# secondmind-labs/markovflow

Hardware: AMD Instinct MI355X
Metric: Kalman log-lik steps/sec (BxT) at d=6 (higher is better)
Workload: dtype f64; 1 GPU; KalmanFilter.log_likelihood B=1024/GPU T=10000 d=6 m=1 f64 (sum of two Matern-5/2, north-star target config); series_per_gpu=1024, state_dim=6, output_dim=1, parallelism=batch-sharded x1, one scalar RCCL all-reduce

## Files before the change

### markovflow_amd/csrc/mf_head_carry.hpp

```cpp
#pragma once

namespace mf {

template <int ROWB, int UNIT, typename Keep> struct HeadCarry {
    static constexpr int LINE = 128;
    static constexpr int MAXT = 2;
    static constexpr int UG = (ROWB + UNIT - 1) / UNIT;
    static constexpr int STEP = ROWB % LINE;
    static constexpr int cand(int t) {
        int n = 0;
        for (int u = 0; u < UG; ++u)
            if (Keep::keep(u, UNIT) && (u + 1) * UNIT <= LINE - 4) { if (n == t) return u; ++n; }
        return -1;
    }
    static constexpr int count_cand() { int n = 0; while (n < MAXT && cand(n) >= 0) ++n; return n; }
    static constexpr int tail_index(int u) { for (int t = 0; t < count_cand(); ++t) if (cand(t) == u) return t; return -1; }
    static constexpr unsigned carried_units(int r) {
        r &= LINE - 1;
        if (r == 0) return 0u;
        const int room = LINE - r;
        unsigned m = 0u;
        for (int u = 0; u < UG; ++u) {
            if (!Keep::keep(u, UNIT) || u * UNIT >= room) continue;
            const int t = tail_index(u);
            if (t < 0 || (u + 1) * UNIT > room) return 0u;
            m |= 1u << t;
        }
        return m;
    }
    static constexpr unsigned table(int t) {
        unsigned m = 0u;
        for (int g = 0; g < 32; ++g) if ((carried_units(4 * g) >> t) & 1u) m |= 1u << g;
        return m;
    }
    static constexpr unsigned TAB0 = table(0), TAB1 = table(1);
    static constexpr int period() { int p = 1, r = STEP; while (r % LINE) { r += STEP; ++p; } return p; }
    static constexpr int PERIOD = (ROWB % 4 == 0) ? period() : 0;
    static constexpr bool USABLE = ROWB % 4 == 0 && ROWB >= LINE && STEP != 0 && Keep::keep(UG - 1, UNIT) && (TAB0 | TAB1) != 0u;
    static constexpr int NT = USABLE ? count_cand() : 0;
    static constexpr int tail_unit(int t) { return cand(t); }

    static constexpr bool carried(unsigned addr, int t) { return (((t == 0 ? TAB0 : TAB1) >> ((addr & (LINE - 1)) >> 2)) & 1u) != 0u; }

    static constexpr unsigned consumer_bits(unsigned addr0) {
        unsigned m = 0u;
        for (int t = 0; t < NT; ++t)
            for (int p = 0; p < PERIOD; ++p) if (carried(addr0 + (unsigned)(p * STEP), t)) m |= 1u << (t * PERIOD + p);
        return m;
    }
    static constexpr unsigned producer_bits(unsigned addr0, int kind) {
        unsigned m = 0u;
        for (int p = 0; p < PERIOD; ++p) {
            bool f = true;
            if (kind >= 1 + MAXT) f = carried(addr0 + (unsigned)((p + 1) * STEP), kind - 1 - MAXT);
            else if (kind >= 1) f = !carried(addr0 + (unsigned)(p * STEP), kind - 1);
            if (f) m |= 1u << p;
        }
        return m;
    }
};

template <int ROWB, typename Keep, bool TAIL = false> struct Stream {
    static constexpr int UNIT = (ROWB >= 16) ? 16 : 4;
    static constexpr int UG = (ROWB + UNIT - 1) / UNIT;
    static constexpr int count_kept() { int n = 0; for (int u = 0; u < UG; ++u) n += Keep::keep(u, UNIT) ? 1 : 0; return n; }
    using HC = HeadCarry<ROWB, UNIT, Keep>;
    static constexpr int UB = count_kept();
    static constexpr int NT = TAIL ? HC::NT : 0;
    static constexpr int U = UB + NT;
    static constexpr int NI = U;
    static constexpr int LDS_BYTES = 64 * U * UNIT;
    static constexpr bool ALL = (UB == UG) && NT == 0;
    static constexpr int global_unit(int c) {
        int n = 0;
        for (int u = 0; u < UG; ++u) if (Keep::keep(u, UNIT)) { if (n == c) return u; ++n; }
        return -1;
    }
    static constexpr int global_offset(int c) { return c < UB ? global_unit(c) * UNIT : ROWB + HC::tail_unit(c - UB) * UNIT; }
    static constexpr int unit_kind(int c) {
        if (c >= UB) return 1 + HC::MAXT + (c - UB);
        for (int t = 0; t < NT; ++t) if (global_unit(c) == HC::tail_unit(t)) return 1 + t;
        return 0;
    }
    static constexpr int compact_unit(int gu) {
        int n = 0;
        for (int u = 0; u < gu; ++u) n += Keep::keep(u, UNIT) ? 1 : 0;
        return n;
    }
};

struct KeepAll { static constexpr bool keep(int, int) { return true; } };
template <int D, int S> struct KeepLower {
    static constexpr bool keep(int u, int unit) {
        const int lo = u * unit, hi = lo + unit;
        for (int i = 0; i < D; ++i) {
            const int a = (i * D) * S, b = (i * D + i + 1) * S;
            if (a < hi && lo < b) return true;
        }
        return false;
    }
};

}
```

### markovflow_amd/csrc/mf_kf_lds.hpp

```cpp
#pragma once
#include "mf_kernels.hpp"
#include "mf_head_carry.hpp"
#include <type_traits>
#ifndef MF_PUMPMASK
#define MF_PUMPMASK 63
#endif

namespace mf {

typedef int mf_v4i __attribute__((ext_vector_type(4)));

#define MF_POLICY_STR_0 ""
#define MF_POLICY_STR_1 " nt"
#define MF_POLICY_STR_2 " sc1"
#define MF_POLICY_STR_3 " sc0 sc1"
#define MF_POLICY_STR_4 " sc0"
#define MF_POLICY_CAT(n) MF_POLICY_STR_##n
#define MF_POLICY_OF(n) MF_POLICY_CAT(n)
#ifndef MF_POLW
#define MF_POLW 1
#endif
#ifndef MF_POLN
#define MF_POLN 0
#endif
#define MF_POLICY_WIDE MF_POLICY_OF(MF_POLW)
#define MF_POLICY_NARROW MF_POLICY_OF(MF_POLN)
#define MF_DMA_HEAD "s_nop 4\n\ts_mov_b32 %0, m0\n\ts_mov_b32 m0, %2\n\ts_nop 0\n\t"
#define MF_DMA_TAIL "s_mov_b32 m0, %0"
#define MF_DMA_X4(v, pol) "buffer_load_dwordx4 " v ", %1, 0 offen" pol " lds\n\t"
#define MF_DMA_X1(v, pol) "buffer_load_dword " v ", %1, 0 offen" pol " lds\n\t"
#define MF_DMA_STEP4 "s_add_u32 m0, m0, 0x400\n\ts_nop 0\n\t"
#define MF_DMA_STEP1 "s_add_u32 m0, m0, 0x100\n\ts_nop 0\n\t"
template <bool WIDE, int N> MF_DEV void dma_b128_group(mf_v4i srd, unsigned lds_addr, const unsigned* v) {
    unsigned keep;
    static_assert(N >= 1 && N <= 4, "group size");
#define MF_DMA_B128_BODY(POL)                                                                                                       \
    if constexpr (N == 1)                                                                                                           \
        asm volatile(MF_DMA_HEAD MF_DMA_X4("%3", POL) MF_DMA_TAIL : "=&s"(keep) : "s"(srd), "s"(lds_addr), "v"(v[0]) : "memory", "scc"); \
    else if constexpr (N == 2)                                                                                                      \
        asm volatile(MF_DMA_HEAD MF_DMA_X4("%3", POL) MF_DMA_STEP4 MF_DMA_X4("%4", POL) MF_DMA_TAIL                                 \
                     : "=&s"(keep) : "s"(srd), "s"(lds_addr), "v"(v[0]), "v"(v[1]) : "memory", "scc");                              \
    else if constexpr (N == 3)                                                                                                      \
        asm volatile(MF_DMA_HEAD MF_DMA_X4("%3", POL) MF_DMA_STEP4 MF_DMA_X4("%4", POL) MF_DMA_STEP4 MF_DMA_X4("%5", POL) MF_DMA_TAIL \
                     : "=&s"(keep) : "s"(srd), "s"(lds_addr), "v"(v[0]), "v"(v[1]), "v"(v[2]) : "memory", "scc");                   \
    else                                                                                                                            \
        asm volatile(MF_DMA_HEAD MF_DMA_X4("%3", POL) MF_DMA_STEP4 MF_DMA_X4("%4", POL) MF_DMA_STEP4 MF_DMA_X4("%5", POL)           \
                     MF_DMA_STEP4 MF_DMA_X4("%6", POL) MF_DMA_TAIL                                                                  \
                     : "=&s"(keep) : "s"(srd), "s"(lds_addr), "v"(v[0]), "v"(v[1]), "v"(v[2]), "v"(v[3]) : "memory", "scc");
    if (WIDE) { MF_DMA_B128_BODY(MF_POLICY_WIDE) } else { MF_DMA_B128_BODY(MF_POLICY_NARROW) }
#undef MF_DMA_B128_BODY
}
template <int N> MF_DEV void dma_b32_group(mf_v4i srd, unsigned lds_addr, const unsigned* v) {
    unsigned keep;
    static_assert(N >= 1 && N <= 4, "group size");
    if constexpr (N == 1)
        asm volatile(MF_DMA_HEAD MF_DMA_X1("%3", MF_POLICY_NARROW) MF_DMA_TAIL : "=&s"(keep) : "s"(srd), "s"(lds_addr), "v"(v[0]) : "memory", "scc");
    else if constexpr (N == 2)
        asm volatile(MF_DMA_HEAD MF_DMA_X1("%3", MF_POLICY_NARROW) MF_DMA_STEP1 MF_DMA_X1("%4", MF_POLICY_NARROW) MF_DMA_TAIL
                     : "=&s"(keep) : "s"(srd), "s"(lds_addr), "v"(v[0]), "v"(v[1]) : "memory", "scc");
    else if constexpr (N == 3)
        asm volatile(MF_DMA_HEAD MF_DMA_X1("%3", MF_POLICY_NARROW) MF_DMA_STEP1 MF_DMA_X1("%4", MF_POLICY_NARROW) MF_DMA_STEP1
                     MF_DMA_X1("%5", MF_POLICY_NARROW) MF_DMA_TAIL
                     : "=&s"(keep) : "s"(srd), "s"(lds_addr), "v"(v[0]), "v"(v[1]), "v"(v[2]) : "memory", "scc");
    else
        asm volatile(MF_DMA_HEAD MF_DMA_X1("%3", MF_POLICY_NARROW) MF_DMA_STEP1 MF_DMA_X1("%4", MF_POLICY_NARROW) MF_DMA_STEP1
                     MF_DMA_X1("%5", MF_POLICY_NARROW) MF_DMA_STEP1 MF_DMA_X1("%6", MF_POLICY_NARROW) MF_DMA_TAIL
                     : "=&s"(keep) : "s"(srd), "s"(lds_addr), "v"(v[0]), "v"(v[1]), "v"(v[2]), "v"(v[3]) : "memory", "scc");
}


constexpr unsigned MF_DMA_INVALID = 0xF0000000u;
constexpr unsigned long long MF_DMA_MAXREC = 0xE0000000ull;

template <typename St, typename = void> struct StreamTail { static constexpr int NT = 0, PERIOD = 1; };
template <typename St> struct StreamTail<St, std::enable_if_t<(St::NT > 0)>> { static constexpr int NT = St::NT, PERIOD = St::HC::PERIOD; };

template <typename St> struct DmaStream {
    using TL = StreamTail<St>;
    unsigned vo[St::NI];
    static constexpr int PB = TL::PERIOD;
    static constexpr int FW = TL::NT > 0 ? (St::NI * PB + 31) / 32 : 1;
    unsigned fm[FW];
    MF_DEV void init(const char* smem, int lane, int rel_tab, int gtab, unsigned base_lo = 0u) {
        const int q0 = lane / St::U, c0 = lane - q0 * St::U;
        if constexpr (TL::NT > 0) { MF_UNROLL for (int w = 0; w < FW; ++w) fm[w] = 0u; }
        MF_UNROLL for (int i = 0; i < St::NI; ++i) {
            const int a = (64 * i) / St::U, b = (64 * i) % St::U;
            int cu = c0 + b;
            const int carry = cu >= St::U ? 1 : 0;
            cu -= carry * St::U;
            const int row = q0 + a + carry;
            const unsigned rel = *reinterpret_cast<const unsigned*>(smem + rel_tab + row * 4);
            unsigned off;
            if (St::ALL) off = (unsigned)cu * St::UNIT;
            else off = *reinterpret_cast<const unsigned*>(smem + gtab + cu * 4);
            vo[i] = rel + off;
            if constexpr (TL::NT > 0) {
                static_assert(PB < 32 && 32 % PB == 0, "an instruction's schedule bits do not straddle two words");
                int kind = 0;
                MF_UNROLL for (int cc = 0; cc < St::U; ++cc) if (St::unit_kind(cc) != 0 && cu == cc) kind = St::unit_kind(cc);
                unsigned bits = (1u << PB) - 1u;
                MF_UNROLL for (int kk = 1; kk <= 2 * St::HC::MAXT; ++kk)
                    if (kind == kk) bits = St::HC::producer_bits(base_lo + rel, kk);
                fm[(i * PB) / 32] |= bits << ((i * PB) % 32);
            }
#ifdef MF_EXPERIMENT
            if (pack_base != 0xffffffffu && rel < MF_DMA_INVALID)
                vo[i] |= ((((pack_base + rel) >> 5) & 3u) << 29) | ((unsigned)(off / St::UNIT) << 24);
#endif
        }
    }
#ifdef MF_EXPERIMENT
    unsigned pack_base = 0xffffffffu;
    unsigned step_next = 0;
    bool skip_carried = false;
    MF_DEV unsigned exp_offset(unsigned v) const {
        if (pack_base == 0xffffffffu || v >= MF_DMA_INVALID) return v;
        const unsigned phase = ((v >> 29) + step_next) & 3u, gu = (v >> 24) & 31u, off = v & 0xffffffu;
        const bool carried = skip_carried && phase != 0u && gu < 8u - 2u * phase;
        return carried ? MF_DMA_INVALID : off;
    }
#endif
    template <int I0, int I1, bool SCHED = false> MF_DEV void issue(mf_v4i srd, unsigned lds_base, unsigned phase = 0u) const {
        constexpr int HI = I1 < St::NI ? I1 : St::NI;
        if constexpr (I0 < HI) {
            constexpr int N = (HI - I0) < 4 ? (HI - I0) : 4;
            unsigned voff[N];
            MF_UNROLL for (int k = 0; k < N; ++k) {
#ifdef MF_EXPERIMENT
                voff[k] = exp_offset(vo[I0 + k]);
#else
                voff[k] = vo[I0 + k];
#endif
                if constexpr (SCHED && TL::NT > 0)
                    voff[k] = ((fm[((I0 + k) * PB) / 32] >> (((I0 + k) * PB) % 32 + phase)) & 1u) ? voff[k] : MF_DMA_INVALID;
            }
            if (St::UNIT == 16) dma_b128_group<(St::UG >= 8), N>(srd, lds_base + I0 * 1024, voff);
            else dma_b32_group<N>(srd, lds_base + I0 * 256, voff);
            issue<I0 + N, I1, SCHED>(srd, lds_base, phase);
        }
    }
};

MF_DEV unsigned long long uniform64(unsigned long long x) {
    const unsigned lo = (unsigned)__builtin_amdgcn_readfirstlane((int)(unsigned)x);
    const unsigned hi = (unsigned)__builtin_amdgcn_readfirstlane((int)(unsigned)(x >> 32));
    return ((unsigned long long)hi << 32) | lo;
}

MF_DEV mf_v4i make_srd(unsigned long long base, unsigned long long end, int debug = 0) {
    unsigned long long rem = end > base ? end - base : 0ull;
    if (debug & 1) rem = 0;
    if (rem > MF_DMA_MAXREC) rem = MF_DMA_MAXREC;
    mf_v4i srd;
    srd.x = __builtin_amdgcn_readfirstlane((int)(unsigned)base);
    srd.y = __builtin_amdgcn_readfirstlane((int)((unsigned)(base >> 32) & 0xffffu));
    srd.z = __builtin_amdgcn_readfirstlane((int)(unsigned)rem);
    srd.w = 0x00020000;
    return srd;
}

template <typename T, typename St> struct RowReader {
    const char* row;
    MF_DEV RowReader(const char* smem, int lds_off, int lane) : row(smem + lds_off + lane * (St::U * St::UNIT)) {}
    MF_DEV T at(int e) const {
        const int byte = e * (int)sizeof(T);
        const int gu = byte / St::UNIT;
        const int off = St::compact_unit(gu) * St::UNIT + (byte - gu * St::UNIT);
        return *reinterpret_cast<const T*>(row + off);
    }
    MF_DEV T tail_at(int t, int k) const { return *reinterpret_cast<const T*>(row + (St::UB + t) * St::UNIT + k * (int)sizeof(T)); }
};

template <typename T, int D, int M, bool RSTEP = false, int BG = 1, bool CARRY = false> struct KfLdsCfg {
    static constexpr int S = sizeof(T);
    static constexpr int BGRP = BG;
    using StA = Stream<D * D * S, KeepAll>;
    using StC0 = Stream<D * D * S, KeepLower<D, S>>;
    using StCT = Stream<D * D * S, KeepLower<D, S>, true>;
    using Stb = Stream<BG * D * S, KeepAll>;
    using StH = Stream<BG * M * D * S, KeepAll>;
    static constexpr int YG = (M == 1) ? 4 : 1;
    using Sty = Stream<YG * M * S, KeepAll>;
    using StR = Stream<M * M * S, KeepAll>;
    static constexpr bool RS = RSTEP;
    static constexpr int QUARTER_CU = (160 * 1024) / 4;
    static constexpr int TABLE_BYTES = 5 * 256 + ((StCT::U * 4 + 15) / 16) * 16;
    static constexpr int IMAGE_T = StA::LDS_BYTES + StCT::LDS_BYTES + Stb::LDS_BYTES + StH::LDS_BYTES + ((Sty::LDS_BYTES + 15) / 16) * 16 +
                                   (RSTEP ? ((StR::LDS_BYTES + 15) / 16) * 16 : 0);
    static constexpr bool TAIL = CARRY && StCT::NT > 0 && !StC0::ALL && StCT::NI * StCT::HC::PERIOD <= 64 &&
                                 StCT::NT * StCT::HC::PERIOD <= 32 && IMAGE_T <= QUARTER_CU && TABLE_BYTES <= IMAGE_T &&
                                 (StA::NI + StCT::NI + Stb::NI + StH::NI + Sty::NI + (RSTEP ? StR::NI : 0)) < 64;
    using StC = Stream<D * D * S, KeepLower<D, S>, TAIL>;
    static constexpr int OFF_A = 0;
    static constexpr int OFF_C = OFF_A + StA::LDS_BYTES;
    static constexpr int OFF_b = OFF_C + StC::LDS_BYTES;
    static constexpr int OFF_H = OFF_b + Stb::LDS_BYTES;
    static constexpr int OFF_y = OFF_H + StH::LDS_BYTES;
    static constexpr int OFF_R = OFF_y + ((Sty::LDS_BYTES + 15) / 16) * 16;
    static constexpr int IMAGE_END = OFF_R + (RSTEP ? ((StR::LDS_BYTES + 15) / 16) * 16 : 0);
    static constexpr int OFF_relA = TAIL ? 0 : IMAGE_END;
    static constexpr int OFF_relb = OFF_relA + 256;
    static constexpr int OFF_relH = OFF_relb + 256;
    static constexpr int OFF_rely = OFF_relH + 256;
    static constexpr int OFF_relR = OFF_rely + 256;
    static constexpr int OFF_gtabC = OFF_relR + 256;
    static constexpr int LDS_TOTAL = TAIL ? IMAGE_END : OFF_gtabC + ((StC::U * 4 + 15) / 16) * 16;
    static constexpr bool SUPPORTED =
                                      (StA::NI + StC::NI + Stb::NI + StH::NI + Sty::NI + (RSTEP ? StR::NI : 0)) < 64 &&
                                      LDS_TOTAL <= 64 * 1024;
};

template <typename T, int D, int M, bool RSTEP = false> using KfChunkCfg = KfLdsCfg<T, D, M, RSTEP, 1, true>;
static_assert(KfChunkCfg<double, 6, 1>::TAIL && KfChunkCfg<double, 6, 1>::LDS_TOTAL <= 40960, "fp64 d = 6: four wavefronts per CU");

template <typename Cfg> struct KfPump {
    static constexpr int N_SMALL = Cfg::StC::NI + Cfg::Stb::NI + Cfg::StH::NI + Cfg::Sty::NI + (Cfg::RS ? Cfg::StR::NI : 0);
    static constexpr int N_BIG = Cfg::StA::NI;
    const DmaStream<typename Cfg::StA>& dA; const DmaStream<typename Cfg::StC>& dC;
    const DmaStream<typename Cfg::Stb>& db; const DmaStream<typename Cfg::StH>& dH;
    const DmaStream<typename Cfg::Sty>& dy; const DmaStream<typename Cfg::StR>& dR;
    mf_v4i sA, sC, sb, sH, sy, sR;
    unsigned lds0;
    bool more;
    bool yfetch = true;
    unsigned cphase = 0;
    template <int K> MF_DEV void small() const {
        if (!((MF_PUMPMASK >> K) & 1)) return;
        small_do<K>();
    }
    template <int K> MF_DEV void small_do() const {
        if (!more) return;
        constexpr int HC = (Cfg::StC::NI + 1) / 2;
        if (K == 0) dC.template issue<0, HC, true>(sC, lds0 + Cfg::OFF_C, cphase);
        else {
            dC.template issue<HC, 64, true>(sC, lds0 + Cfg::OFF_C, cphase);
            db.template issue<0, 64>(sb, lds0 + Cfg::OFF_b);
            dH.template issue<0, 64>(sH, lds0 + Cfg::OFF_H);
            if (yfetch) dy.template issue<0, 64>(sy, lds0 + Cfg::OFF_y);
            if (Cfg::RS) dR.template issue<0, 64>(sR, lds0 + Cfg::OFF_R);
        }
    }
    template <int K> MF_DEV void all() const {
        dC.template issue<0, 64>(sC, lds0 + Cfg::OFF_C);
        db.template issue<0, 64>(sb, lds0 + Cfg::OFF_b);
        dH.template issue<0, 64>(sH, lds0 + Cfg::OFF_H);
        dy.template issue<0, 64>(sy, lds0 + Cfg::OFF_y);
        if (Cfg::RS) dR.template issue<0, 64>(sR, lds0 + Cfg::OFF_R);
        dA.template issue<0, 64>(sA, lds0 + Cfg::OFF_A);
    }
    template <int K> MF_DEV void big() const {
        if (!((MF_PUMPMASK >> (K + 2)) & 1)) return;
        big_do<K>();
    }
    MF_DEV void unpumped() const {
        if (!((MF_PUMPMASK >> 0) & 1)) small_do<0>();
        if (!((MF_PUMPMASK >> 1) & 1)) small_do<1>();
        if (!((MF_PUMPMASK >> 2) & 1)) big_do<0>();
        if (!((MF_PUMPMASK >> 3) & 1)) big_do<1>();
        if (!((MF_PUMPMASK >> 4) & 1)) big_do<2>();
        if (!((MF_PUMPMASK >> 5) & 1)) big_do<3>();
    }
    template <int K> MF_DEV void big_do() const {
        if (!more) return;
        constexpr int Q = (Cfg::StA::NI + 3) / 4;
        dA.template issue<K * Q, (K + 1) * Q>(sA, lds0 + Cfg::OFF_A);
    }
};

template <typename T, int D, int M, bool SPIKE, bool FIRST, typename Pump>
MF_DEV void kf_lds_step(Elim<T, D, SPIKE>& E, LogAcc<T>& laC, T& acc_yry, T& acc_ww, const T (&C)[D][D],
                        const T (&mvec)[D], const T (&hk)[M * D], const T (&yk)[M], const T (&Rsh)[M * M],
                        T (&Bm)[D][D], const Pump& pump, bool active, bool sep_lane) {
    const bool sep = FIRST && sep_lane, ord = active && !sep;
    T Ci[D][D], w[D], btw[D];
    if (active) {
        tri_inv_lower<T, D>(C, Ci, laC, E.bad);
        laC.renorm();
    }
    pump.template small<0>();
    if (active) {
        trimul_lower_vec<T, D>(Ci, mvec, w);
        acc_ww += dot_self<T, D>(w);
    }
    pump.template small<1>();
    pump.template big<0>();
    if (active) {
        trimul_lower_inplace<T, D, D>(Ci, Bm);
        gemv_t<T, D, D>(Bm, w, btw);
    }
    pump.template big<1>();
    if (FIRST && active && sep) {
        syrk_tn_lower<T, D, D>(Bm, E.GU, T(1));
        MF_UNROLL for (int i = 0; i < D; ++i) E.gU[i] = -btw[i];
    }
    if (ord) {
        syrk_tn_lower<T, D, D>(Bm, E.Phi, T(1));
        MF_UNROLL for (int i = 0; i < D; ++i) E.t[i] -= btw[i];
    }
    pump.template big<2>();
    if (FIRST && active && sep) {
        neg_trimulT_lower_inplace<T, D, D>(Ci, Bm);
        MF_UNROLL for (int i = 0; i < D; ++i) MF_UNROLL for (int j = 0; j < D; ++j) E.X[i][j] = Bm[i][j];
    }
    if (ord) E.eliminate_main();
    pump.template big<3>();
    if (FIRST && active && sep) {
        trimulT_self_lower<T, D>(Ci, E.Phi);
        trimulT_lower_vec<T, D>(Ci, w, E.t);
        acc_yry += Obs<T, D, M>::apply(hk, yk, Rsh, M, E.Phi, E.t);
    }
    if (ord) {
        E.eliminate_spike();
        trsm_right_lower_t<T, D, D>(E.Phi, E.Li, Bm);
        neg_trimulT_lower_inplace<T, D, D>(Ci, Bm);
        T Dn[D][D], rn[D];
        trimulT_self_lower<T, D>(Ci, Dn);
        trimulT_lower_vec<T, D>(Ci, w, rn);
        acc_yry += Obs<T, D, M>::apply(hk, yk, Rsh, M, Dn, rn);
        E.advance(Bm, Dn, rn);
    }
}

template <typename T, int D, int M, bool SPIKE, bool RSTEP = false>
__global__ void __launch_bounds__(64) kf_chunk_lds_kernel(KfArgs<T> a, long L, RedSys<T> out) {
    using Cfg = KfChunkCfg<T, D, M, RSTEP>;
    extern __shared__ __attribute__((aligned(16))) char smem[];
    const int lane = threadIdx.x;
    const long total = a.B * a.P;
    const long id_raw = (long)blockIdx.x * 64 + lane;
    const bool valid = id_raw < total;
    const long id = valid ? id_raw : total - 1;
    const long s = id / a.P, c = id % a.P;
    const long nt = a.Tn - 1;
    const long tau0 = c * L;
    long len = nt - tau0;
    if (len > L) len = L;
    if (len < 0 || !valid) len = 0;
    constexpr int S = sizeof(T);

    const unsigned long long offA = (unsigned long long)(s * nt + tau0) * (D * D * S);
    const unsigned long long offb = (unsigned long long)(s * nt + tau0) * (D * S);
    const unsigned long long offH = (unsigned long long)(s * a.Tn + tau0 + 1) * (M * D * S);
    const unsigned long long offy = (unsigned long long)(s * a.Tn + tau0 + 1) * (M * S);
    const unsigned long long offR = (unsigned long long)(s * a.Tn + tau0 + 1) * (M * M * S);
    const unsigned long long offA0 = uniform64(offA), offb0 = uniform64(offb);
    const unsigned long long offH0 = uniform64(offH), offy0 = uniform64(offy), offR0 = uniform64(offR);
    const bool rowok = valid && len > 0;
    {
        unsigned* tab = reinterpret_cast<unsigned*>(smem);
        tab[Cfg::OFF_relA / 4 + lane] = rowok ? (unsigned)(offA - offA0) : MF_DMA_INVALID;
        tab[Cfg::OFF_relb / 4 + lane] = rowok ? (unsigned)(offb - offb0) : MF_DMA_INVALID;
        tab[Cfg::OFF_relH / 4 + lane] = rowok ? (unsigned)(offH - offH0) : MF_DMA_INVALID;
        tab[Cfg::OFF_rely / 4 + lane] = rowok ? (unsigned)(offy - offy0) : MF_DMA_INVALID;
        tab[Cfg::OFF_relR / 4 + lane] = rowok ? (unsigned)(offR - offR0) : MF_DMA_INVALID;
        if (lane < Cfg::StC::U) {
            unsigned g = 0;
            MF_UNROLL for (int cc = 0; cc < Cfg::StC::U; ++cc) if (lane == cc) g = (unsigned)Cfg::StC::global_offset(cc);
            tab[Cfg::OFF_gtabC / 4 + lane] = g;
        }
    }
    DmaStream<typename Cfg::StA> dA;
    DmaStream<typename Cfg::StC> dC;
    DmaStream<typename Cfg::Stb> db;
    DmaStream<typename Cfg::StH> dH;
    DmaStream<typename Cfg::Sty> dy;
    DmaStream<typename Cfg::StR> dR;
    unsigned long long pA = (unsigned long long)a.A + offA0, pC = (unsigned long long)a.cholQ + offA0;
    unsigned long long pb = (unsigned long long)a.b + offb0, pH = (unsigned long long)a.H + offH0;
    unsigned long long py = (unsigned long long)a.y + offy0;
    unsigned long long pR = (unsigned long long)a.Rinv + (RSTEP ? offR0 : 0ull);
    const unsigned long long eA = (unsigned long long)a.A + (unsigned long long)a.B * nt * (D * D * S);
    const unsigned long long eC = (unsigned long long)a.cholQ + (unsigned long long)a.B * nt * (D * D * S);
    const unsigned long long eb = (unsigned long long)a.b + (unsigned long long)a.B * nt * (D * S);
    const unsigned long long eH = (unsigned long long)a.H + (unsigned long long)a.B * a.Tn * (M * D * S);
    const unsigned long long ey = (unsigned long long)a.y + (unsigned long long)a.B * a.Tn * (M * S);
    const unsigned long long eR = (unsigned long long)a.Rinv + (RSTEP ? (unsigned long long)a.B * a.Tn * (M * M * S) : 0ull);
    const unsigned lds0 = (unsigned)(size_t)smem;

    Elim<T, D, SPIKE> E;
    E.init();
    LogAcc<T> laC;
    laC.init();
    T acc_yry = T(0), acc_ww = T(0);
    T Rsh[M * M];
    MF_UNROLL for (int i = 0; i < M * M; ++i) Rsh[i] = RSTEP ? (valid ? a.Rinv[(s * a.Tn) * M * M + i] : T(0)) : a.Rinv[i];
    if (valid && c == 0) {
        T C[D][D], Ci[D][D], mvec[D], w[D];
        load_lower<T, D>(a.cholP0 + s * D * D, C);
        load_vec<T, D>(a.mu0 + s * D, mvec);
        tri_inv_lower<T, D>(C, Ci, laC, E.bad);
        laC.renorm();
        trimul_lower_vec<T, D>(Ci, mvec, w);
        acc_ww += dot_self<T, D>(w);
        trimulT_self_lower<T, D>(Ci, E.Phi);
        trimulT_lower_vec<T, D>(Ci, w, E.t);
        acc_yry += Obs<T, D, M>::apply(a.H + (s * a.Tn) * M * D, a.y + (s * a.Tn) * M, Rsh, M, E.Phi, E.t);
    }

    long nsteps = len;
    MF_UNROLL for (int off = 32; off > 0; off >>= 1) {
        const long o = __shfl_xor((long long)nsteps, off);
        nsteps = o > nsteps ? o : nsteps;
    }
    nsteps = __builtin_amdgcn_readfirstlane((int)nsteps);
    asm volatile("s_waitcnt vmcnt(0) lgkmcnt(0)" ::: "memory");
#ifdef MF_EXPERIMENT
    if (a.debug & 8) {
        dA.pack_base = (unsigned)__builtin_amdgcn_readfirstlane((int)(unsigned)pA);
        dC.pack_base = (unsigned)__builtin_amdgcn_readfirstlane((int)(unsigned)pC);
    }
#endif
    dA.init(smem, lane, Cfg::OFF_relA, 0);
    dC.init(smem, lane, Cfg::OFF_relA, Cfg::OFF_gtabC, (unsigned)pC);
    db.init(smem, lane, Cfg::OFF_relb, 0);
    dH.init(smem, lane, Cfg::OFF_relH, 0);
    dy.init(smem, lane, Cfg::OFF_rely, 0);
    if (RSTEP) dR.init(smem, lane, Cfg::OFF_relR, 0);
    asm volatile("s_waitcnt lgkmcnt(0)" ::: "memory");
    using HC = typename Cfg::StC::HC;
    constexpr int NTAIL = Cfg::StC::NT, CPER = NTAIL > 0 ? HC::PERIOD : 1, UEL = Cfg::StC::UNIT / S;
    const unsigned cbits = NTAIL > 0 ? HC::consumer_bits((unsigned)((unsigned long long)a.cholQ + offA)) : 0u;
    T cv[NTAIL > 0 ? NTAIL : 1][UEL];
    MF_UNROLL for (int t = 0; t < (NTAIL > 0 ? NTAIL : 1); ++t) MF_UNROLL for (int k = 0; k < UEL; ++k) cv[t][k] = T(0);

    const RowReader<T, typename Cfg::StA> rA(smem, Cfg::OFF_A, lane);
    const RowReader<T, typename Cfg::StC> rC(smem, Cfg::OFF_C, lane);
    const RowReader<T, typename Cfg::Stb> rb(smem, Cfg::OFF_b, lane);
    const RowReader<T, typename Cfg::StH> rH(smem, Cfg::OFF_H, lane);
    const RowReader<T, typename Cfg::Sty> ry(smem, Cfg::OFF_y, lane);
    const RowReader<T, typename Cfg::StR> rR(smem, Cfg::OFF_R, lane);

    using Pump = KfPump<Cfg>;

    if (nsteps > 0) {
        Pump p0{dA, dC, db, dH, dy, dR, make_srd(pA, eA, a.debug), make_srd(pC, eC, a.debug | ((a.debug >> 2) & 1)),
                make_srd(pb, eb, a.debug | ((a.debug >> 1) & 1)), make_srd(pH, eH, a.debug | ((a.debug >> 1) & 1)),
                make_srd(py, ey, a.debug | ((a.debug >> 1) & 1)), make_srd(pR, eR, a.debug | ((a.debug >> 1) & 1)), lds0, true};
        p0.template all<0>();
    }

#ifdef MF_STAMP
#define MF_STAMP_AT(var) { unsigned long long t_; asm volatile("s_memtime %0\n\ts_waitcnt lgkmcnt(0)" : "=s"(t_) :: "memory"); var = t_; }
    unsigned long long st_wait = 0, st_io = 0, st_comp = 0, ts0 = 0, ts1 = 0, ts2 = 0, ts3 = 0;
#define MF_STAMP_ACC { asm volatile("" :: "v"(E.quad), "v"(E.Phi[0][0]) : "memory"); MF_STAMP_AT(ts3) st_wait += ts1 - ts0; st_io += ts2 - ts1; st_comp += ts3 - ts2; }
#else
#define MF_STAMP_AT(var)
#define MF_STAMP_ACC
#endif
#ifdef MF_CHECKSUM
    T cs_A = 0, cs_C = 0, cs_b = 0, cs_H = 0, cs_y = 0;
#define MF_CHECKSUM_ACC if (j < len) { MF_UNROLL for (int i = 0; i < D; ++i) { cs_b += mvec[i]; MF_UNROLL for (int jj = 0; jj < D; ++jj) { cs_A += Bm[i][jj] * T(1 + i * D + jj); if (jj <= i) cs_C += C[i][jj] * T(1 + i * D + jj); } } \
        MF_UNROLL for (int i = 0; i < M * D; ++i) cs_H += hk[i] * T(1 + i); MF_UNROLL for (int i = 0; i < M; ++i) cs_y += yk[i]; }
#else
#define MF_CHECKSUM_ACC
#endif
#ifdef MF_EXPERIMENT
#define MF_EXP_STEP_NEXT { dA.step_next = dC.step_next = (unsigned)(j + 1); dA.skip_carried = dC.skip_carried = (a.debug & 8) != 0; }
#else
#define MF_EXP_STEP_NEXT
#endif
#define MF_NOPUMP_ISSUE pump.unpumped();
#define MF_KF_LDS_STEP(FIRST)                                                                                         \
    {                                                                                                                 \
        MF_STAMP_AT(ts0)                                                                                              \
        asm volatile("s_waitcnt vmcnt(0)" ::: "memory");                                                              \
        MF_STAMP_AT(ts1)                                                                                              \
        const bool more = (j + 1 < nsteps);                                                                           \
        const bool yfetch = ((j + 1) % Cfg::YG) == 0;                                                                 \
        pA += D * D * S; pC += D * D * S; pb += D * S; pH += M * D * S; if (RSTEP) pR += M * M * S;                   \
        if (yfetch) py += Cfg::YG * M * S;                                                                            \
        T C[D][D], mvec[D], hk[M * D], yk[M];                                                                         \
        MF_UNROLL for (int i = 0; i < D; ++i) MF_UNROLL for (int jj = 0; jj <= i; ++jj) C[i][jj] = rC.at(i * D + jj); \
        if constexpr (NTAIL > 0) {                                                                                    \
               \
               \
            MF_UNROLL for (int t = 0; t < NTAIL; ++t) {                                                               \
                const bool got = !(FIRST) && ((cbits >> (t * CPER + (int)(j & (CPER - 1)))) & 1u) != 0u;              \
                MF_UNROLL for (int i = 0; i < D; ++i) MF_UNROLL for (int jj = 0; jj <= i; ++jj)                       \
                    if (((i * D + jj) * S) / Cfg::StC::UNIT == HC::tail_unit(t))                                      \
                        C[i][jj] = got ? cv[t][(i * D + jj) - HC::tail_unit(t) * UEL] : C[i][jj];                     \
                MF_UNROLL for (int k = 0; k < UEL; ++k) cv[t][k] = rC.tail_at(t, k);                                  \
            }                                                                                                         \
        }                                                                                                             \
        MF_UNROLL for (int i = 0; i < D; ++i) mvec[i] = rb.at(i);                                                     \
        MF_UNROLL for (int i = 0; i < M * D; ++i) hk[i] = rH.at(i);                                                   \
        MF_UNROLL for (int i = 0; i < M; ++i)                                                                         \
            yk[i] = *reinterpret_cast<const T*>(ry.row + ((int)(j % Cfg::YG) * M + i) * (int)sizeof(T));              \
        if (RSTEP) { MF_UNROLL for (int i = 0; i < M * M; ++i) Rsh[i] = rR.at(i); }                                    \
        T Bm[D][D];                                                                                                   \
        MF_UNROLL for (int i = 0; i < D; ++i) MF_UNROLL for (int jj = 0; jj < D; ++jj) Bm[i][jj] = rA.at(i * D + jj); \
        asm volatile("s_waitcnt lgkmcnt(0)" ::: "memory");                                                            \
        MF_CHECKSUM_ACC                                                                                               \
        MF_STAMP_AT(ts2)                                                                                              \
        const Pump pump{dA, dC, db, dH, dy, dR, make_srd(pA, eA, a.debug),                                            \
                        make_srd(pC, eC, a.debug | ((a.debug >> 2) & 1)),                                             \
                        make_srd(pb, eb, a.debug | ((a.debug >> 1) & 1)),                                             \
                        make_srd(pH, eH, a.debug | ((a.debug >> 1) & 1)),                                             \
                        make_srd(py, ey, a.debug | ((a.debug >> 1) & 1)),                                             \
                        make_srd(pR, eR, a.debug | ((a.debug >> 1) & 1)), lds0, more, yfetch,                         \
                        (unsigned)((j + 1) & (CPER - 1))};                                                            \
        MF_EXP_STEP_NEXT                                                                                              \
        MF_NOPUMP_ISSUE                                                                                               \
        const bool active = j < len;                                                                                  \
        kf_lds_step<T, D, M, SPIKE, FIRST>(E, laC, acc_yry, acc_ww, C, mvec, hk, yk, Rsh, Bm, pump, active, c > 0);    \
        if (E.bad && first_bad < 0) first_bad = tau0 + j;                                                             \
        MF_STAMP_ACC                                                                                                  \
    }
    long j = 0;
    long first_bad = -1;
    if (nsteps > 0) MF_KF_LDS_STEP(true)
    for (j = 1; j < nsteps; ++j) MF_KF_LDS_STEP(false)
#undef MF_KF_LDS_STEP
    asm volatile("s_waitcnt vmcnt(0)" ::: "memory");
    if (valid) {
        const T scalar = T(-0.5) * (acc_yry + acc_ww) + T(0.5) * E.quad - laC.value() - E.laL.value();
        store_chunk<T, D, SPIKE>(out, id, E, scalar);
        if (E.bad && a.info) raise_pivot(a.info, s * a.Tn + (first_bad < 0 ? tau0 : first_bad));
#ifdef MF_CHECKSUM
        out.GU[id * D * D + 0] = cs_A; out.GU[id * D * D + 1] = cs_C; out.GU[id * D * D + 2] = cs_b;
        out.gU[id * D + 0] = cs_H; out.gU[id * D + 1] = cs_y;
#endif
#ifdef MF_STAMP
        if (lane == 0) {
            out.GU[id * D * D + 0] = (T)st_wait; out.GU[id * D * D + 1] = (T)st_io; out.GU[id * D * D + 2] = (T)st_comp;
        }
#endif
    }
}

}
```

Before: 7.840 billion steps/s.

## Carry A-stream tail units, fetch y into registers, defer H DMA past compute

Enables head-carry tail units for the A transition stream as well as the Cholesky stream, so A rows that spill across cache lines are reused from the previous step's tail instead of being refetched. In the tail configuration, observations y are loaded straight into registers with buffer loads instead of going through LDS. H's DMA issue is moved to after the step's compute via a new late() hook. Scalar bookkeeping (first_bad, the loop bound) is narrowed to int and the output id is recomputed after the loop, to cut register pressure in the fp64 d=6 kernel. The aim is fewer LDS bytes and less DMA traffic per step, at the cost of more complex fetch-phase logic and extra VGPRs for y.

```diff
diff --git a/markovflow_amd/csrc/mf_head_carry.hpp b/markovflow_amd/csrc/mf_head_carry.hpp
--- a/markovflow_amd/csrc/mf_head_carry.hpp
+++ b/markovflow_amd/csrc/mf_head_carry.hpp
@@ -77,6 +77,8 @@
         return -1;
     }
     static constexpr int global_offset(int c) { return c < UB ? global_unit(c) * UNIT : ROWB + HC::tail_unit(c - UB) * UNIT; }
+    static constexpr bool linear() { for (int c = 0; c < U; ++c) if (global_offset(c) != c * UNIT) return false; return true; }
+    static constexpr bool LINEAR = linear();
     static constexpr int unit_kind(int c) {
         if (c >= UB) return 1 + HC::MAXT + (c - UB);
         for (int t = 0; t < NT; ++t) if (global_unit(c) == HC::tail_unit(t)) return 1 + t;
diff --git a/markovflow_amd/csrc/mf_kf_lds.hpp b/markovflow_amd/csrc/mf_kf_lds.hpp
--- a/markovflow_amd/csrc/mf_kf_lds.hpp
+++ b/markovflow_amd/csrc/mf_kf_lds.hpp
@@ -74,6 +74,8 @@
 
 template <typename St, typename = void> struct StreamTail { static constexpr int NT = 0, PERIOD = 1; };
 template <typename St> struct StreamTail<St, std::enable_if_t<(St::NT > 0)>> { static constexpr int NT = St::NT, PERIOD = St::HC::PERIOD; };
+template <typename St, typename = void> struct StreamLinear { static constexpr bool value = St::ALL; };
+template <typename St> struct StreamLinear<St, std::void_t<decltype(St::LINEAR)>> { static constexpr bool value = St::LINEAR; };
 
 template <typename St> struct DmaStream {
     using TL = StreamTail<St>;
@@ -92,7 +94,7 @@
             const int row = q0 + a + carry;
             const unsigned rel = *reinterpret_cast<const unsigned*>(smem + rel_tab + row * 4);
             unsigned off;
-            if (St::ALL) off = (unsigned)cu * St::UNIT;
+            if (StreamLinear<St>::value) off = (unsigned)cu * St::UNIT;
             else off = *reinterpret_cast<const unsigned*>(smem + gtab + cu * 4);
             vo[i] = rel + off;
             if constexpr (TL::NT > 0) {
@@ -160,6 +162,36 @@
     return srd;
 }
 
+MF_DEV __amdgpu_buffer_rsrc_t make_rsrc(unsigned long long base, unsigned long long end, int debug = 0) {
+    unsigned long long rem = end > base ? end - base : 0ull;
+    if (debug & 1) rem = 0;
+    if (rem > MF_DMA_MAXREC) rem = MF_DMA_MAXREC;
+    return __builtin_amdgcn_make_buffer_rsrc(reinterpret_cast<void*>(uniform64(base)),
+                                             (short)0, __builtin_amdgcn_readfirstlane((int)(unsigned)rem), 0x00020000);
+}
+
+template <typename T, int N> MF_DEV void buffer_load_group(__amdgpu_buffer_rsrc_t r, unsigned voff, T (&v)[N]) {
+    typedef unsigned v4u __attribute__((ext_vector_type(4)));
+    typedef unsigned v2u __attribute__((ext_vector_type(2)));
+    constexpr int NW = N * (int)sizeof(T) / 4;
+    static_assert((N * sizeof(T)) % 4 == 0, "whole dwords");
+    constexpr int N4 = NW / 4, O2 = 4 * N4, O1 = O2 + ((NW % 4) >= 2 ? 2 : 0);
+    unsigned w[NW];
+    MF_UNROLL for (int q = 0; q < N4; ++q) {
+        const v4u x = __builtin_amdgcn_raw_buffer_load_b128(r, (int)(voff + 16u * q), 0, 0);
+        w[4 * q] = x.x; w[4 * q + 1] = x.y; w[4 * q + 2] = x.z; w[4 * q + 3] = x.w;
+    }
+    if constexpr (O1 > O2) {
+        const v2u x = __builtin_amdgcn_raw_buffer_load_b64(r, (int)(voff + 4u * O2), 0, 0);
+        w[O2] = x.x; w[O2 + 1] = x.y;
+    }
+    if constexpr (NW > O1) w[O1] = __builtin_amdgcn_raw_buffer_load_b32(r, (int)(voff + 4u * O1), 0, 0);
+    MF_UNROLL for (int i = 0; i < N; ++i) {
+        if constexpr (sizeof(T) == 8) v[i] = __builtin_bit_cast(T, ((unsigned long long)w[2 * i + 1] << 32) | w[2 * i]);
+        else v[i] = __builtin_bit_cast(T, w[i]);
+    }
+}
+
 template <typename T, typename St> struct RowReader {
     const char* row;
     MF_DEV RowReader(const char* smem, int lds_off, int lane) : row(smem + lds_off + lane * (St::U * St::UNIT)) {}
@@ -172,10 +204,24 @@
     MF_DEV T tail_at(int t, int k) const { return *reinterpret_cast<const T*>(row + (St::UB + t) * St::UNIT + k * (int)sizeof(T)); }
 };
 
+template <typename T, typename St, bool LOWER, int ROWS, int COLS, int NTAIL, int UEL>
+MF_DEV void take_carried(const RowReader<T, St>& rd, unsigned bits, bool first, long j, T (&X)[ROWS][COLS], T (&cv)[NTAIL][UEL]) {
+    using HC = typename St::HC;
+    constexpr int PER = HC::PERIOD;
+    MF_UNROLL for (int t = 0; t < St::NT; ++t) {
+        const bool got = !first && ((bits >> (t * PER + (int)(j & (PER - 1)))) & 1u) != 0u;
+        MF_UNROLL for (int i = 0; i < ROWS; ++i) MF_UNROLL for (int jj = 0; jj < (LOWER ? i + 1 : COLS); ++jj)
+            if (((i * COLS + jj) * (int)sizeof(T)) / St::UNIT == HC::tail_unit(t))
+                X[i][jj] = got ? cv[t][(i * COLS + jj) - HC::tail_unit(t) * UEL] : X[i][jj];
+        MF_UNROLL for (int k = 0; k < UEL; ++k) cv[t][k] = rd.tail_at(t, k);
+    }
+}
+
 template <typename T, int D, int M, bool RSTEP = false, int BG = 1, bool CARRY = false> struct KfLdsCfg {
     static constexpr int S = sizeof(T);
     static constexpr int BGRP = BG;
-    using StA = Stream<D * D * S, KeepAll>;
+    using StA0 = Stream<D * D * S, KeepAll>;
+    using StAT = Stream<D * D * S, KeepAll, true>;
     using StC0 = Stream<D * D * S, KeepLower<D, S>>;
     using StCT = Stream<D * D * S, KeepLower<D, S>, true>;
     using Stb = Stream<BG * D * S, KeepAll>;
@@ -186,18 +232,22 @@
     static constexpr bool RS = RSTEP;
     static constexpr int QUARTER_CU = (160 * 1024) / 4;
     static constexpr int TABLE_BYTES = 5 * 256 + ((StCT::U * 4 + 15) / 16) * 16;
-    static constexpr int IMAGE_T = StA::LDS_BYTES + StCT::LDS_BYTES + Stb::LDS_BYTES + StH::LDS_BYTES + ((Sty::LDS_BYTES + 15) / 16) * 16 +
+    static constexpr int Y_LDS = ((Sty::LDS_BYTES + 15) / 16) * 16;
+    static constexpr int IMAGE_T = StAT::LDS_BYTES + StCT::LDS_BYTES + Stb::LDS_BYTES + StH::LDS_BYTES +
                                    (RSTEP ? ((StR::LDS_BYTES + 15) / 16) * 16 : 0);
     static constexpr bool TAIL = CARRY && StCT::NT > 0 && !StC0::ALL && StCT::NI * StCT::HC::PERIOD <= 64 &&
-                                 StCT::NT * StCT::HC::PERIOD <= 32 && IMAGE_T <= QUARTER_CU && TABLE_BYTES <= IMAGE_T &&
-                                 (StA::NI + StCT::NI + Stb::NI + StH::NI + Sty::NI + (RSTEP ? StR::NI : 0)) < 64;
+                                 StCT::NT * StCT::HC::PERIOD <= 32 &&
+                                 (StAT::NT == 0 || (StAT::LINEAR && StAT::NT * StAT::HC::PERIOD <= 32)) &&
+                                 IMAGE_T <= QUARTER_CU && TABLE_BYTES <= IMAGE_T &&
+                                 (StAT::NI + StCT::NI + Stb::NI + StH::NI + Sty::NI + (RSTEP ? StR::NI : 0)) < 64;
+    using StA = Stream<D * D * S, KeepAll, TAIL>;
     using StC = Stream<D * D * S, KeepLower<D, S>, TAIL>;
     static constexpr int OFF_A = 0;
     static constexpr int OFF_C = OFF_A + StA::LDS_BYTES;
     static constexpr int OFF_b = OFF_C + StC::LDS_BYTES;
     static constexpr int OFF_H = OFF_b + Stb::LDS_BYTES;
     static constexpr int OFF_y = OFF_H + StH::LDS_BYTES;
-    static constexpr int OFF_R = OFF_y + ((Sty::LDS_BYTES + 15) / 16) * 16;
+    static constexpr int OFF_R = OFF_y + (TAIL ? 0 : Y_LDS);
     static constexpr int IMAGE_END = OFF_R + (RSTEP ? ((StR::LDS_BYTES + 15) / 16) * 16 : 0);
     static constexpr int OFF_relA = TAIL ? 0 : IMAGE_END;
     static constexpr int OFF_relb = OFF_relA + 256;
@@ -213,6 +263,7 @@
 
 template <typename T, int D, int M, bool RSTEP = false> using KfChunkCfg = KfLdsCfg<T, D, M, RSTEP, 1, true>;
 static_assert(KfChunkCfg<double, 6, 1>::TAIL && KfChunkCfg<double, 6, 1>::LDS_TOTAL <= 40960, "fp64 d = 6: four wavefronts per CU");
+static_assert(KfChunkCfg<double, 6, 1>::StA::NT == 2 && KfChunkCfg<double, 6, 1>::StC::NT == 2, "fp64 d = 6: both wide streams carry");
 
 template <typename Cfg> struct KfPump {
     static constexpr int N_SMALL = Cfg::StC::NI + Cfg::Stb::NI + Cfg::StH::NI + Cfg::Sty::NI + (Cfg::RS ? Cfg::StR::NI : 0);
@@ -236,16 +287,23 @@
         else {
             dC.template issue<HC, 64, true>(sC, lds0 + Cfg::OFF_C, cphase);
             db.template issue<0, 64>(sb, lds0 + Cfg::OFF_b);
-            dH.template issue<0, 64>(sH, lds0 + Cfg::OFF_H);
-            if (yfetch) dy.template issue<0, 64>(sy, lds0 + Cfg::OFF_y);
+            if constexpr (!Cfg::TAIL) {
+                dH.template issue<0, 64>(sH, lds0 + Cfg::OFF_H);
+                if (yfetch) dy.template issue<0, 64>(sy, lds0 + Cfg::OFF_y);
+            }
             if (Cfg::RS) dR.template issue<0, 64>(sR, lds0 + Cfg::OFF_R);
         }
+    }
+    MF_DEV void late() const {
+        asm volatile("s_waitcnt lgkmcnt(0)" ::: "memory");
+        if (!more) return;
+        dH.template issue<0, 64>(sH, lds0 + Cfg::OFF_H);
     }
     template <int K> MF_DEV void all() const {
         dC.template issue<0, 64>(sC, lds0 + Cfg::OFF_C);
         db.template issue<0, 64>(sb, lds0 + Cfg::OFF_b);
         dH.template issue<0, 64>(sH, lds0 + Cfg::OFF_H);
-        dy.template issue<0, 64>(sy, lds0 + Cfg::OFF_y);
+        if constexpr (!Cfg::TAIL) dy.template issue<0, 64>(sy, lds0 + Cfg::OFF_y);
         if (Cfg::RS) dR.template issue<0, 64>(sR, lds0 + Cfg::OFF_R);
         dA.template issue<0, 64>(sA, lds0 + Cfg::OFF_A);
     }
@@ -264,13 +322,42 @@
     template <int K> MF_DEV void big_do() const {
         if (!more) return;
         constexpr int Q = (Cfg::StA::NI + 3) / 4;
-        dA.template issue<K * Q, (K + 1) * Q>(sA, lds0 + Cfg::OFF_A);
+        dA.template issue<K * Q, (K + 1) * Q, true>(sA, lds0 + Cfg::OFF_A, cphase);
     }
 };
 
-template <typename T, int D, int M, bool SPIKE, bool FIRST, typename Pump>
+template <typename T, int D, int M> struct ObsRegs {
+    T hk[M * D], yk[M];
+    MF_DEV void get(T (&h)[M * D], T (&y)[M]) const {
+        MF_UNROLL for (int i = 0; i < M * D; ++i) h[i] = hk[i];
+        MF_UNROLL for (int i = 0; i < M; ++i) y[i] = yk[i];
+    }
+};
+template <typename T, int D, int M, typename Cfg> struct ObsEarly : ObsRegs<T, D, M> {
+    MF_DEV ObsEarly(const RowReader<T, typename Cfg::StH>& rH, const char* yrow, const T (&)[Cfg::YG * M], long j) {
+        MF_UNROLL for (int i = 0; i < M * D; ++i) this->hk[i] = rH.at(i);
+        MF_UNROLL for (int i = 0; i < M; ++i)
+            this->yk[i] = *reinterpret_cast<const T*>(yrow + ((int)(j % Cfg::YG) * M + i) * (int)sizeof(T));
+    }
+};
+template <typename T, int D, int M, typename Cfg> struct ObsLate {
+    const RowReader<T, typename Cfg::StH> rH;
+    T yg[Cfg::YG * M];
+    const int ysel;
+    MF_DEV ObsLate(const RowReader<T, typename Cfg::StH>& rH_, const char*, const T (&yg_)[Cfg::YG * M], long j)
+        : rH(rH_), ysel((int)(j % Cfg::YG)) { MF_UNROLL for (int i = 0; i < Cfg::YG * M; ++i) yg[i] = yg_[i]; }
+    MF_DEV void get(T (&h)[M * D], T (&y)[M]) const {
+        MF_UNROLL for (int i = 0; i < M * D; ++i) h[i] = rH.at(i);
+        MF_UNROLL for (int i = 0; i < M; ++i) {
+            y[i] = yg[i];
+            MF_UNROLL for (int g = 1; g < Cfg::YG; ++g) y[i] = ysel == g ? yg[g * M + i] : y[i];
+        }
+    }
+};
+
+template <typename T, int D, int M, bool SPIKE, bool FIRST, typename Pump, typename ObsSrc>
 MF_DEV void kf_lds_step(Elim<T, D, SPIKE>& E, LogAcc<T>& laC, T& acc_yry, T& acc_ww, const T (&C)[D][D],
-                        const T (&mvec)[D], const T (&hk)[M * D], const T (&yk)[M], const T (&Rsh)[M * M],
+                        const T (&mvec)[D], const ObsSrc& obs, const T (&Rsh)[M * M],
                         T (&Bm)[D][D], const Pump& pump, bool active, bool sep_lane) {
     const bool sep = FIRST && sep_lane, ord = active && !sep;
     T Ci[D][D], w[D], btw[D];
@@ -308,6 +395,8 @@
     if (FIRST && active && sep) {
         trimulT_self_lower<T, D>(Ci, E.Phi);
         trimulT_lower_vec<T, D>(Ci, w, E.t);
+        T hk[M * D], yk[M];
+        obs.get(hk, yk);
         acc_yry += Obs<T, D, M>::apply(hk, yk, Rsh, M, E.Phi, E.t);
     }
     if (ord) {
@@ -317,9 +406,21 @@
         T Dn[D][D], rn[D];
         trimulT_self_lower<T, D>(Ci, Dn);
         trimulT_lower_vec<T, D>(Ci, w, rn);
+        T hk[M * D], yk[M];
+        obs.get(hk, yk);
         acc_yry += Obs<T, D, M>::apply(hk, yk, Rsh, M, Dn, rn);
         E.advance(Bm, Dn, rn);
     }
+}
+
+template <typename T, int D, int M, bool SPIKE, bool FIRST, typename Pump>
+MF_DEV void kf_lds_step(Elim<T, D, SPIKE>& E, LogAcc<T>& laC, T& acc_yry, T& acc_ww, const T (&C)[D][D],
+                        const T (&mvec)[D], const T (&hk)[M * D], const T (&yk)[M], const T (&Rsh)[M * M],
+                        T (&Bm)[D][D], const Pump& pump, bool active, bool sep_lane) {
+    ObsRegs<T, D, M> obs;
+    MF_UNROLL for (int i = 0; i < M * D; ++i) obs.hk[i] = hk[i];
+    MF_UNROLL for (int i = 0; i < M; ++i) obs.yk[i] = yk[i];
+    kf_lds_step<T, D, M, SPIKE, FIRST>(E, laC, acc_yry, acc_ww, C, mvec, obs, Rsh, Bm, pump, active, sep_lane);
 }
 
 template <typename T, int D, int M, bool SPIKE, bool RSTEP = false>
@@ -347,6 +448,7 @@
     const unsigned long long offA0 = uniform64(offA), offb0 = uniform64(offb);
     const unsigned long long offH0 = uniform64(offH), offy0 = uniform64(offy), offR0 = uniform64(offR);
     const bool rowok = valid && len > 0;
+    const int ilen = (int)len;
     {
         unsigned* tab = reinterpret_cast<unsigned*>(smem);
         tab[Cfg::OFF_relA / 4 + lane] = rowok ? (unsigned)(offA - offA0) : MF_DMA_INVALID;
@@ -411,18 +513,27 @@
         dC.pack_base = (unsigned)__builtin_amdgcn_readfirstlane((int)(unsigned)pC);
     }
 #endif
-    dA.init(smem, lane, Cfg::OFF_relA, 0);
+    dA.init(smem, lane, Cfg::OFF_relA, 0, (unsigned)pA);
     dC.init(smem, lane, Cfg::OFF_relA, Cfg::OFF_gtabC, (unsigned)pC);
     db.init(smem, lane, Cfg::OFF_relb, 0);
     dH.init(smem, lane, Cfg::OFF_relH, 0);
-    dy.init(smem, lane, Cfg::OFF_rely, 0);
+    if constexpr (!Cfg::TAIL) dy.init(smem, lane, Cfg::OFF_rely, 0);
     if (RSTEP) dR.init(smem, lane, Cfg::OFF_relR, 0);
     asm volatile("s_waitcnt lgkmcnt(0)" ::: "memory");
     using HC = typename Cfg::StC::HC;
+    using HCA = typename Cfg::StA::HC;
     constexpr int NTAIL = Cfg::StC::NT, CPER = NTAIL > 0 ? HC::PERIOD : 1, UEL = Cfg::StC::UNIT / S;
+    constexpr int NTA = Cfg::StA::NT, UELA = Cfg::StA::UNIT / S;
+    static_assert(NTA == 0 || (NTAIL > 0 && HCA::PERIOD == HC::PERIOD), "one fetch phase (KfPump::cphase) serves both streams");
     const unsigned cbits = NTAIL > 0 ? HC::consumer_bits((unsigned)((unsigned long long)a.cholQ + offA)) : 0u;
-    T cv[NTAIL > 0 ? NTAIL : 1][UEL];
+    const unsigned abits = NTA > 0 ? HCA::consumer_bits((unsigned)((unsigned long long)a.A + offA)) : 0u;
+    T cv[NTAIL > 0 ? NTAIL : 1][UEL], av[NTA > 0 ? NTA : 1][UELA];
     MF_UNROLL for (int t = 0; t < (NTAIL > 0 ? NTAIL : 1); ++t) MF_UNROLL for (int k = 0; k < UEL; ++k) cv[t][k] = T(0);
+    MF_UNROLL for (int t = 0; t < (NTA > 0 ? NTA : 1); ++t) MF_UNROLL for (int k = 0; k < UELA; ++k) av[t][k] = T(0);
+    T yg[Cfg::YG * M];
+    MF_UNROLL for (int i = 0; i < Cfg::YG * M; ++i) yg[i] = T(0);
+    const unsigned rely = rowok ? (unsigned)(offy - offy0) : MF_DMA_INVALID;
+    using ObsSrc = std::conditional_t<Cfg::TAIL, ObsLate<T, D, M, Cfg>, ObsEarly<T, D, M, Cfg>>;
 
     const RowReader<T, typename Cfg::StA> rA(smem, Cfg::OFF_A, lane);
     const RowReader<T, typename Cfg::StC> rC(smem, Cfg::OFF_C, lane);
@@ -438,6 +549,7 @@
                 make_srd(pb, eb, a.debug | ((a.debug >> 1) & 1)), make_srd(pH, eH, a.debug | ((a.debug >> 1) & 1)),
                 make_srd(py, ey, a.debug | ((a.debug >> 1) & 1)), make_srd(pR, eR, a.debug | ((a.debug >> 1) & 1)), lds0, true};
         p0.template all<0>();
+        if constexpr (Cfg::TAIL) buffer_load_group(make_rsrc(py, ey, a.debug | ((a.debug >> 1) & 1)), rely, yg);
     }
 
 #ifdef MF_STAMP
@@ -450,9 +562,11 @@
 #endif
 #ifdef MF_CHECKSUM
     T cs_A = 0, cs_C = 0, cs_b = 0, cs_H = 0, cs_y = 0;
+#define MF_CHECKSUM_HK T hk[M * D], yk[M]; obs.get(hk, yk);
 #define MF_CHECKSUM_ACC if (j < len) { MF_UNROLL for (int i = 0; i < D; ++i) { cs_b += mvec[i]; MF_UNROLL for (int jj = 0; jj < D; ++jj) { cs_A += Bm[i][jj] * T(1 + i * D + jj); if (jj <= i) cs_C += C[i][jj] * T(1 + i * D + jj); } } \
         MF_UNROLL for (int i = 0; i < M * D; ++i) cs_H += hk[i] * T(1 + i); MF_UNROLL for (int i = 0; i < M; ++i) cs_y += yk[i]; }
 #else
+#define MF_CHECKSUM_HK
 #define MF_CHECKSUM_ACC
 #endif
 #ifdef MF_EXPERIMENT
@@ -465,32 +579,23 @@
     {                                                                                                                 \
         MF_STAMP_AT(ts0)                                                                                              \
         asm volatile("s_waitcnt vmcnt(0)" ::: "memory");                                                              \
+        if constexpr (Cfg::TAIL) { MF_UNROLL for (int i = 0; i < Cfg::YG * M; ++i) asm volatile("" : "+v"(yg[i])); }  \
         MF_STAMP_AT(ts1)                                                                                              \
         const bool more = (j + 1 < nsteps);                                                                           \
         const bool yfetch = ((j + 1) % Cfg::YG) == 0;                                                                 \
         pA += D * D * S; pC += D * D * S; pb += D * S; pH += M * D * S; if (RSTEP) pR += M * M * S;                   \
         if (yfetch) py += Cfg::YG * M * S;                                                                            \
-        T C[D][D], mvec[D], hk[M * D], yk[M];                                                                         \
+        T C[D][D], mvec[D];                                                                                           \
         MF_UNROLL for (int i = 0; i < D; ++i) MF_UNROLL for (int jj = 0; jj <= i; ++jj) C[i][jj] = rC.at(i * D + jj); \
-        if constexpr (NTAIL > 0) {                                                                                    \
-               \
-               \
-            MF_UNROLL for (int t = 0; t < NTAIL; ++t) {                                                               \
-                const bool got = !(FIRST) && ((cbits >> (t * CPER + (int)(j & (CPER - 1)))) & 1u) != 0u;              \
-                MF_UNROLL for (int i = 0; i < D; ++i) MF_UNROLL for (int jj = 0; jj <= i; ++jj)                       \
-                    if (((i * D + jj) * S) / Cfg::StC::UNIT == HC::tail_unit(t))                                      \
-                        C[i][jj] = got ? cv[t][(i * D + jj) - HC::tail_unit(t) * UEL] : C[i][jj];                     \
-                MF_UNROLL for (int k = 0; k < UEL; ++k) cv[t][k] = rC.tail_at(t, k);                                  \
-            }                                                                                                         \
-        }                                                                                                             \
+        if constexpr (NTAIL > 0) take_carried<T, typename Cfg::StC, true>(rC, cbits, FIRST, j, C, cv);                \
         MF_UNROLL for (int i = 0; i < D; ++i) mvec[i] = rb.at(i);                                                     \
-        MF_UNROLL for (int i = 0; i < M * D; ++i) hk[i] = rH.at(i);                                                   \
-        MF_UNROLL for (int i = 0; i < M; ++i)                                                                         \
-            yk[i] = *reinterpret_cast<const T*>(ry.row + ((int)(j % Cfg::YG) * M + i) * (int)sizeof(T));              \
+        const ObsSrc obs(rH, ry.row, yg, j);                                                                          \
         if (RSTEP) { MF_UNROLL for (int i = 0; i < M * M; ++i) Rsh[i] = rR.at(i); }                                    \
         T Bm[D][D];                                                                                                   \
         MF_UNROLL for (int i = 0; i < D; ++i) MF_UNROLL for (int jj = 0; jj < D; ++jj) Bm[i][jj] = rA.at(i * D + jj); \
+        if constexpr (NTA > 0) take_carried<T, typename Cfg::StA, false>(rA, abits, FIRST, j, Bm, av);                \
         asm volatile("s_waitcnt lgkmcnt(0)" ::: "memory");                                                            \
+        MF_CHECKSUM_HK                                                                                                \
         MF_CHECKSUM_ACC                                                                                               \
         MF_STAMP_AT(ts2)                                                                                              \
         const Pump pump{dA, dC, db, dH, dy, dR, make_srd(pA, eA, a.debug),                                            \
@@ -502,21 +607,31 @@
                         (unsigned)((j + 1) & (CPER - 1))};                                                            \
         MF_EXP_STEP_NEXT                                                                                              \
         MF_NOPUMP_ISSUE                                                                                               \
-        const bool active = j < len;                                                                                  \
-        kf_lds_step<T, D, M, SPIKE, FIRST>(E, laC, acc_yry, acc_ww, C, mvec, hk, yk, Rsh, Bm, pump, active, c > 0);    \
-        if (E.bad && first_bad < 0) first_bad = tau0 + j;                                                             \
+        const bool active = (int)j < ilen;                                                                            \
+        kf_lds_step<T, D, M, SPIKE, FIRST>(E, laC, acc_yry, acc_ww, C, mvec, obs, Rsh, Bm, pump, active, c > 0);      \
+        if constexpr (Cfg::TAIL) {                                                                                    \
+            pump.late();                                                                                              \
+            if (more && yfetch)                                                                                       \
+                buffer_load_group(make_rsrc(py, ey, a.debug | ((a.debug >> 1) & 1)),                                  \
+                                  (int)j + 1 < ilen ? rely : MF_DMA_INVALID, yg);                                           \
+        }                                                                                                             \
+        if (E.bad && first_bad < 0) first_bad = (int)j;                                                               \
         MF_STAMP_ACC                                                                                                  \
     }
     long j = 0;
-    long first_bad = -1;
+    int first_bad = -1;
     if (nsteps > 0) MF_KF_LDS_STEP(true)
     for (j = 1; j < nsteps; ++j) MF_KF_LDS_STEP(false)
 #undef MF_KF_LDS_STEP
     asm volatile("s_waitcnt vmcnt(0)" ::: "memory");
-    if (valid) {
+    int lane_e = lane;
+    if constexpr (Cfg::TAIL) asm volatile("" : "+v"(lane_e));
+    const long id_e = (long)blockIdx.x * 64 + lane_e;
+    if (id_e < total) {
+        const long id = id_e, s = id / a.P, tau0 = (id % a.P) * L;
         const T scalar = T(-0.5) * (acc_yry + acc_ww) + T(0.5) * E.quad - laC.value() - E.laL.value();
         store_chunk<T, D, SPIKE>(out, id, E, scalar);
-        if (E.bad && a.info) raise_pivot(a.info, s * a.Tn + (first_bad < 0 ? tau0 : first_bad));
+        if (E.bad && a.info) raise_pivot(a.info, s * a.Tn + tau0 + (first_bad < 0 ? 0 : first_bad));
 #ifdef MF_CHECKSUM
         out.GU[id * D * D + 0] = cs_A; out.GU[id * D * D + 1] = cs_C; out.GU[id * D * D + 2] = cs_b;
         out.gU[id * D + 0] = cs_H; out.gU[id * D + 1] = cs_y;
```

Result: no change. 7.816 billion steps/s (-0.3%).
